# goldbricklemon/uplift-upsample-3dhpe

Measured on AMD Instinct MI355X. Metric: pose-sequences/sec, higher is better.
Workload: dtype f16x3 (f32 operands split into f16 hi/lo, 3 MFMA passes, f32 accumulate); 1 GPU; config/h36m_351.json forward, N=71 tokens (receptive field 351), J=17, batch 128/GPU, s_in=5, seeded Keras-default weights; global_batch=128, parallelism=batch-sharded x1, hipgraph=True, concurrent_half_batches=False, batches_in_flight=8

## Files before the change

uplift-upsample-3dhpe_amd/arch.py:

```python
import math
from dataclasses import dataclass, field
from typing import List, Tuple


@dataclass(frozen=True)
class UpliftArch:
    num_frames: int
    num_keypoints: int
    d_spatial: int
    d_temporal: int
    spatial_depth: int
    temporal_depth: int
    strides: Tuple[int, ...]
    paddings: Tuple[Tuple[int, int], ...]
    num_heads: int
    mlp_ratio: float
    qkv_bias: bool
    has_strided_input: bool
    first_strided_token_attention_layer: int
    full_output: bool
    drop_path_rate: Tuple[float, float, float]
    batch_size: int
    drop_rate: float = 0.0
    attention_drop_rate: float = 0.0
# ... 1 lines not shown
    learnable_masked_token: bool = False
    output_bn: bool = False
    strided_lengths: Tuple[int, ...] = field(default=())

    @property
    def h_spatial(self) -> int:
        return int(self.d_spatial * self.mlp_ratio)

    @property
    def h_temporal(self) -> int:
        return int(self.d_temporal * self.mlp_ratio)

    @property
    def out_dim(self) -> int:
        return 3 * self.num_keypoints

    @property
    def compiled_dims(self) -> bool:
        return (self.num_keypoints == 17 and self.d_spatial == 32 and self.h_spatial == 64 and self.num_heads == 8
                and self.d_temporal == 384)


def _pe_length_recurrence(n: int, strides, paddings) -> List[int]:
    out = [n]
    for s, p in zip(strides, paddings):
        out.append(math.ceil((out[-1] + p[0] + p[1] - 2) / s))
    return out


def _conv_length_recurrence(n: int, strides, paddings) -> List[int]:
    out = [n]
    for s, p in zip(strides, paddings):
        out.append((out[-1] + p[0] + p[1] - 3) // s + 1)
    return out


def training_unsupported(a: "UpliftArch"):
    out = []
    if not (0.0 <= a.drop_rate < 1.0):
        out.append(f"DROP_RATE = {a.drop_rate} (must be in [0, 1))")
    if not (0.0 <= a.attention_drop_rate < 1.0):
        out.append(f"ATTENTION_DROP_RATE = {a.attention_drop_rate} (must be in [0, 1))")
    return out


def arch_from_config(config) -> UpliftArch:
    has_strided_input = config.MASK_STRIDE is not None
    if has_strided_input:
        ms = config.MASK_STRIDE
        if type(ms) is int and ms == 1:
            has_strided_input = False
        if type(ms) is list and ms[0] == 1:
            has_strided_input = False

    strides = tuple(int(s) for s in config.STRIDES)
    if config.PADDINGS is None:
        paddings = tuple((1, 1) for _ in strides)
    else:
        paddings = tuple((int(p[0]), int(p[1])) for p in config.PADDINGS)
    if len(paddings) != len(strides):
        raise ValueError("PADDINGS must have one [left, right] pair per entry of STRIDES")

    n = int(config.SEQUENCE_LENGTH)
    pe_len = _pe_length_recurrence(n, strides, paddings)
    conv_len = _conv_length_recurrence(n, strides, paddings)
    if pe_len[:-1] != conv_len[:-1]:
# ... 68 lines not shown
```

uplift-upsample-3dhpe_amd/csrc/uu3d_api.hip:

```cpp
#include <hip/hip_runtime.h>

#include <algorithm>
#include <cmath>
#include <cstdio>
#include <cstdlib>
#include <cstring>
#include <functional>
#include <map>
#include <mutex>
#include <string>
#include <vector>

#include "../../include/uu3d.h"
#include "uu3d_switches.h"
#include "uu3d_gemm.h"
#include "uu3d_gemm_h3.h"
#include "uu3d_gemm_panel.h"
#include "uu3d_gemm_panel8.h"
#include "uu3d_gemm_wt.h"
#include "uu3d_mlp_fused.h"
#include "uu3d_tchain16.h"
#include "uu3d_attn.h"
#include "uu3d_attn_h3.h"
#include "uu3d_spatial.h"
// ... 37 lines not shown

struct WeightRec {
    std::string name;
    std::vector<int64_t> dims;
    int64_t numel = 0;
    std::vector<float> host;
    bool set = false;
};

struct BlockDev {
    const float *ln1_g, *ln1_b, *wqkv_t, *bqkv, *wp_t, *bp, *ln2_g, *ln2_b, *w1_t, *b1, *w2_t, *b2;
    const float* pe;
    size_t wqkv_pf = 0, w1_pf = 0;
    size_t w2_mf = 0;
    size_t wp_pf = 0;
};

struct ProfRec {
    std::string name, kernel;
    double flops, bytes;
    hipEvent_t e0, e1;
};

}

struct uu3d_train_state;
struct uu3d_model {
    uu3d_config cfg;
    uu3d_train_state* ts = nullptr;
    int device = 0;
    std::vector<WeightRec> weights;
    std::map<std::string, int> index;
    std::vector<int> L;
    Switches sw;
    bool committed = false;
    bool generic = false;
    float* gparams = nullptr;
    float* arena = nullptr;
    size_t arena_floats = 0;
    bool throughput = false;
    struct TcLaunch { int flags; size_t w_off ; size_t p_off ; };
    std::vector<TcLaunch> tchain;
    int num_cus = 256;
    std::recursive_mutex train_mu;
    bool in_commit = false;
    int* d_range = nullptr;
    _Float16* harena = nullptr;
    size_t harena_halfs = 0;
    std::map<size_t, std::pair<size_t, size_t>> hplanes;
    std::map<size_t, size_t> panel_off, mlpf_off;
    SpatialParams sp{};
    size_t sp_frag_off = 0;
    size_t sp_frag16_off = 0;
    const float *s2t_wt = nullptr, *s2t_b = nullptr, *token = nullptr, *pe_t = nullptr;
    std::vector<BlockDev> tblocks, sblocks;
    const float *h1_wt = nullptr, *h1_b = nullptr, *h2_wt = nullptr, *h2_b = nullptr;
    bool profiling = false;
    std::vector<ProfRec> prof;
    size_t prof_used = 0;
    std::string err;
};

namespace {

inline bool tchain_possible(const uu3d_config& c) {
    return c.precision == UU3D_PREC_F16X3 && c.d_temporal == 384 && c.h_temporal == 768 && c.num_heads == 8 && c.temporal_depth >= 1;
// ... 664 lines not shown
```

uplift-upsample-3dhpe_amd/csrc/uu3d_attn.h:

```cpp
#pragma once
#include <hip/hip_runtime.h>
#include <stdint.h>
#include <math.h>
#include "uu3d_gemm.h"

namespace uu3d {

typedef _Float16 h16x8v __attribute__((ext_vector_type(8)));
#ifdef UU3D_ATTN_STAMP
__device__ unsigned long long attn_clk[8];
#define ATTN_STAMP(...) __VA_ARGS__
#else
#define ATTN_STAMP(...)
#endif
template <int NT, int DH, bool SPLIT = false>
__global__ void __launch_bounds__(64 * NT)
attn_f32_kernel(const float* __restrict__ qkv, const int ld, const int D, const int L, const int H,
                const uint8_t* __restrict__ key_mask,
                float* __restrict__ out, const int ldo, const size_t lo_off = 0)
{
    static_assert(DH % 16 == 0, "head dim must be a multiple of 16");
    constexpr int LD = DH + 4;
    constexpr int F4 = DH / 4;
    constexpr int KT = DH / 16;
    constexpr int NS = (16 * F4 + 63) / 64;
    __shared__ __attribute__((aligned(16))) float Ks[NT * 16 * LD];
    __shared__ __attribute__((aligned(16))) float Vs[NT * 16 * LD];
    __shared__ __attribute__((aligned(16))) _Float16 Os[SPLIT ? NT : 1][SPLIT ? 2 * 16 * DH : 8];

    const int tid = threadIdx.x;
    const int lane = tid & 63, w = tid >> 6;
    const int qi = lane & 15, g = lane >> 4;
    const int qrow = 16 * w + qi;
    const int bh = ((int)gridDim.x & 7) == 0 ? ((int)blockIdx.x & 7) * ((int)gridDim.x >> 3) + ((int)blockIdx.x >> 3) : (int)blockIdx.x;

    const int b = bh / H, h = bh - b * H;
    float4 kreg[NS], vreg[NS];
    f32x4 qf[KT];
    {
        const float* base = qkv + (size_t)b * L * ld + h * DH;
#pragma unroll
        for (int s = 0; s < NS; ++s) {
            const int idx = tid + s * 64 * NT;
            const int row = idx / F4, c4 = (idx - row * F4) * 4;
            const float* p = base + (size_t)min(row, L - 1) * ld + c4;
            const float keep = (row < L) ? 1.0f : 0.0f;
            const float4 kv = *reinterpret_cast<const float4*>(p + D), vv = *reinterpret_cast<const float4*>(p + 2 * D);
            kreg[s] = make_float4(kv.x * keep, kv.y * keep, kv.z * keep, kv.w * keep);
            vreg[s] = make_float4(vv.x * keep, vv.y * keep, vv.z * keep, vv.w * keep);
        }
#pragma unroll
        for (int t = 0; t < KT; ++t)
            qf[t] = *reinterpret_cast<const f32x4*>(base + (size_t)min(qrow, L - 1) * ld + 16 * t + 4 * g);
    }
    ATTN_STAMP(const long long c0 = clock64();)
#pragma unroll
    for (int s = 0; s < NS; ++s) {
        const int idx = tid + s * 64 * NT;
        const int row = idx / F4, c4 = (idx - row * F4) * 4;
        if ((16 * F4) % 64 == 0 || idx < NT * 16 * F4) {
            *reinterpret_cast<float4*>(&Ks[row * LD + c4]) = kreg[s];
            *reinterpret_cast<float4*>(&Vs[row * LD + c4]) = vreg[s];
        }
    }
    __syncthreads();
    ATTN_STAMP(const long long c1 = clock64();)

    f32x4 st[NT];
#pragma unroll
    for (int j = 0; j < NT; ++j) {
        f32x4 a = (f32x4){0.f, 0.f, 0.f, 0.f};
// ... 46 lines not shown
    ATTN_STAMP(asm volatile("s_nop 0" :: "v"(st[NT - 1][3])); const long long c3 = clock64();)
    f32x4 ot[KT];
#pragma unroll
    for (int t = 0; t < KT; ++t) ot[t] = (f32x4){0.f, 0.f, 0.f, 0.f};
#pragma unroll
        for (int t = 0; t < KT; ++t)
#pragma unroll
            for (int j = 0; j < NT; ++j)
#pragma unroll
                for (int s = 0; s < 4; ++s) {
                    const float vv = Vs[(16 * j + 4 * g + s) * LD + 16 * t + qi];
                    ot[t] = __builtin_amdgcn_mfma_f32_16x16x4f32(st[j][s], vv, ot[t], 0, 0, 0);
                }
    if constexpr (SPLIT) {
        _Float16* Ow = Os[w];
#pragma unroll
        for (int t = 0; t < KT; ++t)
#pragma unroll
            for (int r = 0; r < 4; ++r) {
                const _Float16 hv = (fabsf(ot[t][r]) < 6.103515625e-05f) ? (_Float16)0.f : (_Float16)ot[t][r];
                const _Float16 lv = (_Float16)((ot[t][r] - (float)hv) * 2048.0f);
                Ow[(4 * g + r) * DH + 16 * t + qi] = hv;
                Ow[(16 + 4 * g + r) * DH + 16 * t + qi] = lv;
            }
        __builtin_amdgcn_fence(__ATOMIC_RELEASE, "wavefront");
        __builtin_amdgcn_wave_barrier();
        constexpr int PPR = DH / 8, PIECES = 2 * 16 * PPR;
        _Float16* oh = reinterpret_cast<_Float16*>(out);
#pragma unroll
        for (int i = 0; i < (PIECES + 63) / 64; ++i) {
            const int pc = lane + 64 * i;
            const int plane = pc / (16 * PPR), rem = pc - plane * 16 * PPR, row = rem / PPR, c8 = rem - row * PPR;
            const int q = 16 * w + row;
            if (pc < PIECES && q < L) {
                const h16x8v piece = *reinterpret_cast<const h16x8v*>(&Ow[(plane * 16 + row) * DH + 8 * c8]);
                const int grow = b * L + q, k = h * DH + 8 * c8;
                _Float16* dst = lo_off == 512 ? oh + ((size_t)(grow >> 5) * (size_t)(ldo >> 4) + (size_t)(k >> 4)) * 1024 + (size_t)plane * 512 + ((k >> 3) & 1) * 256 + (grow & 31) * 8
                                              : oh + (size_t)plane * lo_off + (size_t)grow * ldo + k;
                *reinterpret_cast<h16x8v*>(dst) = piece;
            }
        }
    } else {
#pragma unroll
        for (int t = 0; t < KT; ++t)
#pragma unroll
            for (int r = 0; r < 4; ++r) {
                const int q = 16 * w + 4 * g + r;
                if (q < L) out[((size_t)b * L + q) * ldo + h * DH + 16 * t + qi] = ot[t][r];
            }
    }
    ATTN_STAMP(asm volatile("s_waitcnt vmcnt(0)" ::: "memory"); if (tid == 0) { const long long c4 = clock64();
        atomicAdd(&attn_clk[0], (unsigned long long)(c1 - c0)); atomicAdd(&attn_clk[1], (unsigned long long)(c2 - c1));
        atomicAdd(&attn_clk[2], (unsigned long long)(c3 - c2)); atomicAdd(&attn_clk[3], (unsigned long long)(c4 - c3)); atomicAdd(&attn_clk[4], 1ull); })
}

template <int NT, int DH, bool SPLIT = false>
__global__ void __launch_bounds__(256, 1) __attribute__((amdgpu_waves_per_eu(1, 1)))
attn_head_wave_kernel(const float* __restrict__ qkv, const int ld, const int D, const int L, const int H,
                      const uint8_t* __restrict__ key_mask, float* __restrict__ out, const int ldo, const size_t lo_off, const int items)
{
    static_assert(DH % 16 == 0, "head dim must be a multiple of 16");
    constexpr int LD = DH + 4;
    constexpr int F4 = DH / 4;
    constexpr int KT = DH / 16;
    constexpr int NS = (NT * 16 * F4 + 63) / 64;
    constexpr int OS_HALFS = 2 * 16 * DH;
    extern __shared__ __attribute__((aligned(16))) float attn_lds[];
    const int tid = threadIdx.x, lane = tid & 63, w = tid >> 6;
    const int qi = lane & 15, g = lane >> 4;
    float* Ks = attn_lds + (size_t)w * 2 * NT * 16 * LD;
    float* Vs = Ks + NT * 16 * LD;
    _Float16* Os = reinterpret_cast<_Float16*>(attn_lds + (size_t)4 * 2 * NT * 16 * LD) + w * OS_HALFS;
    const int wg = ((int)gridDim.x & 7) == 0 ? ((int)blockIdx.x & 7) * ((int)gridDim.x >> 3) + ((int)blockIdx.x >> 3) : (int)blockIdx.x;
    const int bh = wg * 4 + w;
    if (bh >= items) return;
    size_t lo_off_s = lo_off; int ldo_s = ldo;
    asm volatile("" : "+s"(lo_off_s), "+s"(ldo_s));
    const int b = bh / H, h = bh - b * H;
    const float* base = qkv + (size_t)b * L * ld + h * DH;
    ATTN_STAMP(const long long c0 = clock64(); long long tqk = 0, tsm = 0, tpv = 0;)

    static_assert((NT * 16 * F4) % 64 == 0, "whole staging passes");
    {
        static_assert(NS <= 15, "the counted waits list at most 15 registers");
        f32x4 kx[15], vx[15];
        auto scalar_ptr = [](const float* q) {
// ... 179 lines not shown
```

uplift-upsample-3dhpe_amd/csrc/uu3d_commit.inc:

```
namespace {

struct Packer {
    std::vector<float> buf;
    std::vector<std::pair<size_t, size_t>> dense;
    size_t alloc(size_t n) {
        size_t off = align_up(buf.size(), 64);
        buf.resize(off + n, 0.f);
        return off;
    }
    size_t alloc_dense(size_t n) { const size_t off = alloc(n); dense.emplace_back(off, n); return off; }
};

const float* W(const uu3d_model* m, const std::string& name) {
    auto it = m->index.find(name);
    return it == m->index.end() ? nullptr : m->weights[it->second].host.data();
}

void pack_dense_t(std::vector<float>& buf, size_t off, const float* w, int K, int N, int Kp, int n0) {
    for (int k = 0; k < K; ++k)
        for (int n = 0; n < N; ++n) buf[off + (size_t)(n0 + n) * Kp + k] = w[(size_t)k * N + n];
}

}

int uu3d_commit_weights(uu3d_model* m, void* stream_) {
    if (!m) return UU3D_ERR_INVALID_ARGUMENT;
    for (auto& r : m->weights)
        if (!r.set) return fail(m, UU3D_ERR_NOT_READY, "weight never set: " + r.name);
    hipStream_t stream = (hipStream_t)stream_;
    HIPCHK(m, hipSetDevice(m->device));
    if (m->generic) {
        if (m->gparams == nullptr) {
            long long n = 0;
            for (auto& r : m->weights) n += r.numel;
            HIPCHK(m, hipMalloc((void**)&m->gparams, (size_t)n * sizeof(float)));
        }
        m->in_commit = true;
        const int r = uu3d_train_init(m, m->gparams, stream_);
        m->in_commit = false;
        if (r != UU3D_OK) return r;
        HIPCHK(m, hipStreamSynchronize(stream));
        m->committed = true;
        return UU3D_OK;
    }
    const uu3d_config& c = m->cfg;
    const int J = c.num_keypoints, N = c.num_frames, ds = c.d_spatial, dt = c.d_temporal, ht = c.h_temporal;
    const int Kdt = round_up(dt, 32), Kht = round_up(ht, 32), Ks2t = round_up(J * ds, 32);
    Packer P;

    const size_t o_ew = P.alloc(2 * ds), o_eb = P.alloc(ds), o_spe = P.alloc((size_t)J * ds);
    std::copy_n(W(m, "keypoint_embedding/kernel"), 2 * ds, P.buf.begin() + o_ew);
    std::copy_n(W(m, "keypoint_embedding/bias"), ds, P.buf.begin() + o_eb);
    std::copy_n(W(m, "spatial_pe/positional_encoding_weights"), J * ds, P.buf.begin() + o_spe);
// ... 292 lines not shown
                tchain16_reorder_mlp(tmp.data(), mlp);
            }
            m->tchain.push_back({tb.flags, at, tb.p_off});
        }
        if (m->harena_halfs < hb.size()) {
            if (m->harena) HIPCHK(m, hipFree(m->harena));
            m->harena = nullptr;
            HIPCHK(m, hipMalloc((void**)&m->harena, hb.size() * sizeof(_Float16)));
            m->harena_halfs = hb.size();
        }
        HIPCHK(m, hipMemcpyAsync(m->harena, hb.data(), hb.size() * sizeof(_Float16), hipMemcpyHostToDevice, stream));
        HIPCHK(m, hipStreamSynchronize(stream));
    }

    const float* A = m->arena;
    m->sp.embed_w = A + o_ew; m->sp.embed_b = A + o_eb; m->sp.pe = A + o_spe; m->sp.blocks = A + o_sblk;
    m->sp.norm_g = A + o_sng; m->sp.norm_b = A + o_snb; m->sp.depth = c.spatial_depth; m->sp.total_frames = 0;
    m->s2t_wt = A + o_s2t; m->s2t_b = A + o_s2tb; m->token = A + o_tok; m->pe_t = A + o_pet;
    auto view = [&](const BlockOff& o, bool strided) {
        BlockDev b{};
        b.ln1_g = A + o.ln1_g; b.ln1_b = A + o.ln1_b; b.wqkv_t = A + o.wqkv; b.bqkv = A + o.bqkv;
        b.wp_t = A + o.wp; b.bp = A + o.bp; b.ln2_g = A + o.ln2_g; b.ln2_b = A + o.ln2_b;
        b.w1_t = A + o.w1; b.b1 = A + o.b1; b.w2_t = A + o.w2; b.b2 = A + o.b2;
        b.pe = strided ? A + o.pe : nullptr;
        { const auto it = m->panel_off.find(o.wqkv); b.wqkv_pf = (it != m->panel_off.end()) ? it->second : 0; }
        { const auto it = m->panel_off.find(o.w1); b.w1_pf = (it != m->panel_off.end()) ? it->second : 0; }
        { const auto it = m->mlpf_off.find(o.w2); b.w2_mf = (!strided && it != m->mlpf_off.end()) ? it->second : 0; }
        { const auto it = m->panel_off.find(o.wp); b.wp_pf = (it != m->panel_off.end()) ? it->second : 0; }
        return b;
    };
    m->tblocks.clear(); m->sblocks.clear();
    for (auto& o : toff) m->tblocks.push_back(view(o, false));
    for (auto& o : soff) m->sblocks.push_back(view(o, true));
    m->h1_wt = has_h1 ? A + o_h1 : nullptr; m->h1_b = has_h1 ? A + o_h1b : nullptr;
    m->h2_wt = A + o_h2; m->h2_b = A + o_h2b;
    m->committed = true;
    return UU3D_OK;
}
```

uplift-upsample-3dhpe_amd/csrc/uu3d_forward.inc:

```

namespace {
struct Workspace {
    float *S, *X, *QKV, *O, *Hb, *XA, *XB, *slab, *mslab;
    unsigned char* tc_scratch;
    int* frame_list;
    float2* stats;
    size_t slab_floats;
    size_t bytes;
};
Workspace carve(const uu3d_model* m, int B, char* base) {
    const uu3d_config& c = m->cfg;
    const size_t rows = (size_t)B * c.num_frames;
    const size_t rows_s = (size_t)B * (c.num_strided > 1 ? std::max(m->L[1], 1) : 1);
    size_t off = 0;
    auto take = [&](size_t n) { size_t o = off; off = align_up(off + n, 256); return o; };
    Workspace w{};
    const size_t oS = take(rows * c.num_keypoints * c.d_spatial * 4);
    const size_t oX = take(rows * c.d_temporal * 4);
    const size_t oQ = take((rows + 128) * 3 * c.d_temporal * 4);
    const size_t oO = take((rows + 32) * c.d_temporal * 4);
    const size_t oH = take((rows + 32) * c.h_temporal * 4);
    const size_t oA = take(rows * c.d_temporal * 4);
    const size_t oB = take(rows_s * c.d_temporal * 4);
    const size_t oT = take(rows * sizeof(float2));
// ... 337 lines not shown
            if (nt <= 3) { if (mask) UU3D_ATTN_H3(3, 3, true, nt) else UU3D_ATTN_H3(3, 3, false, nt) }
            else if (nt <= 12) { if (mask) UU3D_ATTN_H3(12, 3, true, nt) else UU3D_ATTN_H3(12, 3, false, nt) }
            else { if (mask) UU3D_ATTN_H3(8, 2, true, std::min(nt, 8)) else UU3D_ATTN_H3(8, 2, false, std::min(nt, 8)) }
#undef UU3D_ATTN_H3
            end();
            return;
        }
        if (!m->sw.attn_wg && H % 4 == 0 && NT >= 4 && NT <= 5) {
            const dim3 hgrid((items + 3) / 4);
#define UU3D_ATTN_HW(nt) case nt: { \
            constexpr size_t lds = attn_head_wave_lds_bytes<nt, kDH>(); \
            if (split_lo_off) { allow_lds<attn_head_wave_kernel<nt, kDH, true>>(lds); \
                hipLaunchKernelGGL((attn_head_wave_kernel<nt, kDH, true>), hgrid, dim3(256), lds, stream, qkv, 3 * D, D, L, H, mask, out, D, frag ? (size_t)512 : split_lo_off, items); } \
            else { allow_lds<attn_head_wave_kernel<nt, kDH, false>>(lds); \
                hipLaunchKernelGGL((attn_head_wave_kernel<nt, kDH, false>), hgrid, dim3(256), lds, stream, qkv, 3 * D, D, L, H, mask, out, D, (size_t)0, items); } \
            } break;
            switch (NT) { UU3D_ATTN_HW(4) UU3D_ATTN_HW(5) default: break; }
#undef UU3D_ATTN_HW
            end();
            return;
        }
#define UU3D_ATTN_CASE(nt) case nt: \
        if (split_lo_off) hipLaunchKernelGGL((attn_f32_kernel<nt, kDH, true>), grid, dim3(64 * nt), 0, stream, qkv, 3 * D, D, L, H, mask, out, D, frag ? (size_t)512 : split_lo_off); \
        else hipLaunchKernelGGL((attn_f32_kernel<nt, kDH, false>), grid, dim3(64 * nt), 0, stream, qkv, 3 * D, D, L, H, mask, out, D, (size_t)0); \
        break;
        switch (NT) {
            UU3D_ATTN_CASE(1) UU3D_ATTN_CASE(2) UU3D_ATTN_CASE(3) UU3D_ATTN_CASE(4)
            UU3D_ATTN_CASE(5) UU3D_ATTN_CASE(6) UU3D_ATTN_CASE(7) UU3D_ATTN_CASE(8)
            default: status = UU3D_ERR_UNSUPPORTED; m->err = "attention over more than 128 tokens needs the f16x3 path (precision f16x3, d_t and h_t multiples of 32)"; break;
        }
#undef UU3D_ATTN_CASE
        end();
    }
};

template <class EP>
void spatial_stage(Launcher& Lh, const uu3d_config& c, const float* kp2d, int M, const uint8_t* mask, int* frame_list, float* S, bool timing_skip, const EP& ep) {
    uu3d_model* const m = Lh.m;
    const int J = c.num_keypoints, ds = c.d_spatial, dt = c.d_temporal;
    const bool h3 = c.precision == UU3D_PREC_F16X3 && !m->sw.spatial_f32 && (m->sw.spatial_h3_always || spatial_h3_pays(M));
    const bool planes = h3 && !m->sw.no_planes && (J * ds) % 32 == 0;
    const bool skip = timing_skip && (skip_mask() & 1);
    SpatialParams sp = m->sp;
    sp.total_frames = M;
    sp.frame_list = nullptr;
    if (mask != nullptr) {
        Lh.begin("compact_frames", "compact_frames", 0.0, (double)M * 5.0);
        hipLaunchKernelGGL(compact_frames_kernel, dim3(1), dim3(1024), 0, Lh.stream, mask, M, frame_list);
        Lh.end();
        sp.frame_list = frame_list;
    }
    const double fl = (double)M * (2.0 * J * 2 * ds + c.spatial_depth * (4.0 * 2 * J * ds * ds + 8.0 * 4 * J * J * (ds / 8) + 2.0 * 2 * J * ds * kHS));
    _Float16* const s_hi = planes ? reinterpret_cast<_Float16*>(S) : (_Float16*)nullptr;
    _Float16* const s_lo = planes ? reinterpret_cast<_Float16*>(S) + (size_t)M * J * ds : (_Float16*)nullptr;
    if (h3 && m->sw.spatial_h3_tiles) {
        Lh.begin("spatial_stack", "spatial_h3", fl, 4.0 * M * J * (2.0 + ds));
        if (!skip)
        hipLaunchKernelGGL((spatial_stack_h3_kernel<kJ, kFR, kSpatialMT>), dim3((M + kFR - 1) / kFR), dim3(64 * (2 / kSpatialMT)), sh3::lds_bytes(), Lh.stream, kp2d, sp,
                           m->harena + m->sp_frag_off, S, s_hi, s_lo, SpatialTrainIO{});
        Lh.end();
    } else if (h3) {
        Lh.begin("spatial_stack", "spatial_p16", fl, 4.0 * M * J * (2.0 + ds));
        if (!skip)
        hipLaunchKernelGGL((spatial_stack_p16_kernel<kJ, kP16FR, kP16PW>), dim3((M + kP16FR - 1) / kP16FR), dim3(64 * p16_waves(kJ, kP16FR, kP16PW)), sp16::lds_bytes<kP16FR>(c.spatial_depth),
                           Lh.stream, kp2d, sp, m->harena + m->sp_frag16_off, S, s_hi, s_lo);
        Lh.end();
// ... 27 lines not shown

struct Forward {
    uu3d_model* const m;
    Launcher Lh;
    const Workspace w;
    const uu3d_config c;
    const uint8_t* const mask;
    const int B;
    float* const full_out; float* const central_out; float* const* const attn_out;
    const bool part_body, part_tail;

    const int N = c.num_frames, J = c.num_keypoints, dt = c.d_temporal, ht = c.h_temporal, M = B * N;
    const bool has_h1 = c.full_output && c.temporal_depth > 0;
    const bool planes = (c.precision == UU3D_PREC_F16X3) && (dt % 32 == 0) && (ht % 32 == 0) && !m->sw.no_planes;
    const bool chain = Lh.throughput && planes && m->sw.tchain_mode != 0 && (m->sw.tchain_mode == 1 || (M + 127) / 128 >= m->sw.tchain_min_tiles) && !m->tchain.empty() && M >= 1024 &&
                       (Lh.attn_is_h3(N, true) || (m->sw.tchain_short && Lh.attn_h3_any(N))) && (c.num_strided == 0 || m->L[0] == N) && (double)M * 1152 * 4.0 < 4.0e9 &&
                       attn_out == nullptr;
    _Float16* const Ph = reinterpret_cast<_Float16*>(w.O);
    _Float16* const Hh = reinterpret_cast<_Float16*>(w.Hb);
    const BlockDev* pend = nullptr;
    float* xa = w.XA;
    char nm[48];

    void tokens_from_frames(const FramesIn& frames) {
        Lh.begin("frames_to_tokens", "frames_to_tokens", 0.0, 4.0 * 3.0 * M * dt);
        hipLaunchKernelGGL(frames_to_tokens_kernel, dim3((unsigned)(((size_t)M * (dt / 4) + 255) / 256)), dim3(256), 0, Lh.stream,
                           frames.features, frames.num_rows, frames.rows, mask, m->token, m->pe_t, (long)M, N, dt, w.X);
        Lh.end();
    }
    void spatial(const float* kp2d) {
        spatial_stage(Lh, c, kp2d, M, mask, w.frame_list, w.S, true, EpSpatialToTemporal{w.X, m->s2t_b, dt, mask, m->token, m->pe_t, N});
    }

    const _Float16* block_head(const char* tag, int i, const BlockDev& b, float* x, int L, const uint8_t* kmask, const BlockDev* prev, bool fuse_mlp) {
        const int Mr = B * L;
        auto name = [&](const char* what) { snprintf(nm, sizeof nm, "%s%d.%s", tag, i + 1, what); return nm; };
        _Float16* const Pl = Ph + (size_t)Mr * dt; _Float16* const Hl = Hh + (size_t)Mr * ht;
        const bool qsplit = Lh.attn_is_h3(L, planes);
        _Float16* const Qh = reinterpret_cast<_Float16*>(w.QKV); _Float16* const Ql = Qh + (size_t)Mr * 3 * dt;
        const EpBiasSplitQ ep_qs{Qh, Ql, b.bqkv, 3 * dt, dt, Lh.attn_qscale()};
        const bool few = planes && Mr <= kFewRows && Lh.wt_ok(b.wqkv_t, dt) && Lh.wt_ok(b.w1_t, dt);
        auto maps = [&]() {
            if (attn_out != nullptr && tag[0] == 't' && attn_out[i] != nullptr) {
                Lh.begin(name("attn_maps"), "attn_probs", 2.0 * B * (double)c.num_heads * L * L * kDH, 4.0 * B * (double)c.num_heads * L * L);
                const size_t lds = (size_t)L * (kDH + 1) * sizeof(float);
                allow_lds<attn_probs_kernel>(160 * 1024 - 256);
                if (qsplit) hipLaunchKernelGGL(attn_probs_kernel, dim3(B * c.num_heads), dim3(256), lds, Lh.stream, (const void*)Qh, (const _Float16*)Ql, 3 * dt, dt, L, c.num_heads, kDH, kmask, 1.0f, 1, attn_out[i]);
                else hipLaunchKernelGGL(attn_probs_kernel, dim3(B * c.num_heads), dim3(256), lds, Lh.stream, (const void*)w.QKV, (const _Float16*)nullptr, 3 * dt, dt, L, c.num_heads, kDH, kmask, 1.0f / sqrtf((float)kDH), 0, attn_out[i]);
                Lh.end();
            }
        };
        if (few) {
            WtLoadF32 l1{x, dt, Mr, dt, b.ln1_g, b.ln1_b, 1e-5f, 1};
            if (qsplit) Lh.gemm_wt(name("ln_qkv"), l1, b.wqkv_t, Mr, 3 * dt, dt, ep_qs);
            else Lh.gemm_wt(name("ln_qkv"), l1, b.wqkv_t, Mr, 3 * dt, dt, EpBias{w.QKV, b.bqkv, 3 * dt});
            maps();
            Lh.attn(name("attn"), w.QKV, B, L, kmask, w.O, (size_t)Mr * dt);
            { GLoadPlain gl{Ph, Pl, dt, Mr}; Lh.gemm_g(name("proj_res"), gl, b.wp_t, Mr, dt, dt, EpBiasResidual{x, b.bp, dt, nullptr, nullptr, 1}, 4.0 * Mr * dt); }
            WtLoadF32 l2{x, dt, Mr, dt, b.ln2_g, b.ln2_b, 1e-5f, 1};
            Lh.gemm_wt(name("ln_fc1"), l2, b.w1_t, Mr, ht, dt, EpBiasReluSplit{Hh, Hl, b.b1, ht});
            return nullptr;
        }
        if (prev != nullptr) {
            if (x == w.X) Lh.ln_res_split_frag(name("ln1_split"), w.X, Mr, prev->b2, w.mslab, nullptr, nullptr, 1, b.ln1_g, b.ln1_b, Ph);
            else Lh.ln_res_split_frag(name("ln1_split"), w.X, Mr, prev->b2, w.mslab, x, b.pe, L, b.ln1_g, b.ln1_b, Ph);
            if (qsplit) Lh.gemm_panel(name("ln_qkv"), Ph, b.wqkv_pf, b.bqkv, Mr, 3 * dt, PanelEpBiasSplitQ{Qh, Ql, 3 * dt, dt, Lh.attn_qscale()});
            else Lh.gemm_panel(name("ln_qkv"), Ph, b.wqkv_pf, b.bqkv, Mr, 3 * dt, PanelEpBias{w.QKV, 3 * dt});
        } else if (planes && Lh.panel_ok(Mr, 3 * dt, dt, b.wqkv_pf)) {
            Lh.ln_split_frag(name("ln1_split"), x, Mr, b.ln1_g, b.ln1_b, Ph);
            if (qsplit) Lh.gemm_panel(name("ln_qkv"), Ph, b.wqkv_pf, b.bqkv, Mr, 3 * dt, PanelEpBiasSplitQ{Qh, Ql, 3 * dt, dt, Lh.attn_qscale()});
            else Lh.gemm_panel(name("ln_qkv"), Ph, b.wqkv_pf, b.bqkv, Mr, 3 * dt, PanelEpBias{w.QKV, 3 * dt});
        } else {
            Lh.row_stats(name("stats1"), x, dt, Mr, w.stats);
            ALoadLayerNorm al{x, w.stats, b.ln1_g, b.ln1_b, dt, Mr, dt};
            if (qsplit) Lh.gemm(name("ln_qkv"), al, b.wqkv_t, Mr, 3 * dt, dt, ep_qs);
            else { EpBias ep{w.QKV, b.bqkv, 3 * dt}; Lh.gemm(name("ln_qkv"), al, b.wqkv_t, Mr, 3 * dt, dt, ep); }
        }
        maps();
        const bool pproj = planes && !m->sw.no_panel_proj && Lh.panel_ok(Mr, dt, dt, b.wp_pf);
        Lh.attn(name("attn"), w.QKV, B, L, kmask, w.O, planes ? (size_t)Mr * dt : 0, pproj);
        const bool mlp_panel = planes && Lh.panel_ok(Mr, ht, dt, b.w1_pf);
        bool ln2_done = false;
        if (pproj) ln2_done = mlp_panel ? Lh.gemm_panel_residual(name("proj_res"), Ph, b.wp_pf, b.bp, Mr, x, b.ln2_g, b.ln2_b, Ph)
                                        : Lh.gemm_panel_residual(name("proj_res"), Ph, b.wp_pf, b.bp, Mr, x);
        else {
            EpBiasResidual ep{x, b.bp, dt, nullptr, nullptr, 1};
            if (planes) { GLoadPlain gl{Ph, Pl, dt, Mr}; Lh.gemm_g(name("proj_res"), gl, b.wp_t, Mr, dt, dt, ep, 4.0 * Mr * dt); }
            else { ALoadPlain al{w.O, dt, Mr, dt}; Lh.gemm(name("proj_res"), al, b.wp_t, Mr, dt, dt, ep, 4.0 * Mr * dt); }
        }
        if (mlp_panel) {
            if (!ln2_done) Lh.ln_split_frag(name("ln2_split"), x, Mr, b.ln2_g, b.ln2_b, Ph);
            if (fuse_mlp) return Ph;
            Lh.gemm_panel(name("ln_fc1"), Ph, b.w1_pf, b.b1, Mr, ht, PanelEpBiasReluSplit{Hh, Hl, ht});
        } else {
            Lh.row_stats(name("stats2"), x, dt, Mr, w.stats);
            ALoadLayerNorm al{x, w.stats, b.ln2_g, b.ln2_b, dt, Mr, dt};
            if (planes) { EpBiasReluSplit ep{Hh, Hl, b.b1, ht}; Lh.gemm(name("ln_fc1"), al, b.w1_t, Mr, ht, dt, ep); }
            else { EpBiasRelu ep{w.Hb, b.b1, ht}; Lh.gemm(name("ln_fc1"), al, b.w1_t, Mr, ht, dt, ep); }
        }
        return nullptr;
    }

    void temporal_chain() {
        _Float16* const Q = reinterpret_cast<_Float16*>(w.QKV);
        Lh.tchain("t1.ln_qkv", m->tchain[0], M, nullptr, w.X, nullptr, nullptr, 1, Q, nullptr, w.tc_scratch);
        for (int i = 0; i < c.temporal_depth; ++i) {
            const bool masked = c.has_strided_input && i < c.first_strided_token_attention_layer;
            snprintf(nm, sizeof nm, "t%d.attn", i + 1);
            Lh.attn(nm, w.QKV, B, N, masked ? mask : nullptr, w.O, (size_t)M * dt, true, true);
            const bool to_strided = i + 1 == c.temporal_depth && c.num_strided > 0;
            snprintf(nm, sizeof nm, "t%d.chain", i + 1);
            Lh.tchain(nm, m->tchain[i + 1], M, Ph, w.X, to_strided ? w.XA : nullptr, to_strided ? m->sblocks[0].pe : nullptr, N, Q, nullptr, w.tc_scratch);
        }
    }
    void temporal_blocks() {
        for (int i = 0; i < c.temporal_depth; ++i) {
            const BlockDev& b = m->tblocks[i];
            const bool masked = c.has_strided_input && i < c.first_strided_token_attention_layer;
            const bool last = (i + 1 == c.temporal_depth);
            const bool fuse = planes && Lh.mlpf_ok(M, b) && (last ? (c.num_strided > 0 && Lh.panel_ok(M, 3 * dt, dt, m->sblocks[0].wqkv_pf))
                                                                  : Lh.panel_ok(M, 3 * dt, dt, m->tblocks[i + 1].wqkv_pf));
            const _Float16* const a2 = block_head("t", i, b, w.X, N, masked ? mask : nullptr, pend, fuse);
            pend = nullptr;
            if (fuse) {
                snprintf(nm, sizeof nm, "t%d.mlp", i + 1);
                Lh.mlp_fused(nm, a2, b, M, w.mslab);
                pend = &b;
                continue;
            }
            const bool to_strided = last && c.num_strided > 0;
            EpBiasResidual ep_fc2{w.X, b.b2, dt, to_strided ? w.XA : nullptr, to_strided ? m->sblocks[0].pe : nullptr, N};
            snprintf(nm, sizeof nm, "t%d.fc2_res", i + 1);
            if (planes) { GLoadPlain gl{Hh, Hh + (size_t)M * ht, ht, M}; Lh.gemm_g(nm, gl, b.w2_t, M, dt, ht, ep_fc2, 4.0 * M * dt); }
            else { ALoadPlain al{w.Hb, ht, M, ht}; Lh.gemm(nm, al, b.w2_t, M, dt, ht, ep_fc2, 4.0 * M * dt); }
        }
    }
    void head1() {
        if (!has_h1) return;
        ALoadPlain al{w.X, dt, M, dt}; EpBias ep{full_out, m->h1_b, 3 * J};
        Lh.gemm("head1", al, m->h1_wt, M, 3 * J, dt, ep);
    }
    void strided_blocks() {
        float* xb = w.XB;
        const _Float16* const hzero = m->harena;
        if (c.temporal_depth == 0 && c.num_strided > 0) {
            Lh.begin("s1.add_pe", "add_pe", 0.0, 12.0 * M * dt);
            hipLaunchKernelGGL(add_period_kernel, dim3((unsigned)(((size_t)M * dt / 4 + 255) / 256)), dim3(256), 0, Lh.stream, w.X, m->sblocks[0].pe, M, dt, N, w.XA);
            Lh.end();
        }
        for (int i = 0; i < c.num_strided; ++i) {
            const BlockDev& b = m->sblocks[i];
            const int Li = m->L[i], Lo = m->L[i + 1], Mi = B * Li, Mo = B * Lo;
            if (((skip_mask() & 256) || part_body) && i >= 1) continue;
            if (((skip_mask() & 512) || part_tail) && i == 0) { std::swap(xa, xb); xb = w.XA; continue; }
            const int lo = (c.strides[i] > 1 && c.pad_left[i] == 0) ? 1 : 0;
            const EpConvResidual ep_conv{xb, b.b2, dt, xa, Li, Lo, c.strides[i], lo,
                                         (i + 1 < c.num_strided) ? m->sblocks[i + 1].pe : nullptr};
            const bool smask = c.temporal_depth == 0 && c.has_strided_input && i < c.first_strided_token_attention_layer;
            if (chain && i == 0) {
                Lh.attn("s1.attn", w.QKV, B, Li, nullptr, w.O, (size_t)Mi * dt, true, true);
                Lh.tchain("s1.chain", m->tchain[c.temporal_depth + 1], Mi, Ph, nullptr, xa, nullptr, 1, nullptr, Hh, w.tc_scratch);
            } else
            block_head("s", i, b, xa, Li, smask ? mask : nullptr, i == 0 ? pend : nullptr, false);
            if (i == 0) head1();
            snprintf(nm, sizeof nm, "s%d.conv_res", i + 1);
            if (planes) { GLoadConv3 gl{Hh, Hh + (size_t)Mi * ht, hzero, ht, Li, Lo, c.strides[i], c.pad_left[i], Mo};
                          Lh.gemm_g(nm, gl, b.w2_t, Mo, dt, 3 * ht, ep_conv, 4.0 * Mo * dt); }
            else { ALoadConv3 al{w.Hb, ht, Li, Lo, c.strides[i], c.pad_left[i], Mo, 3 * ht};
                   Lh.gemm(nm, al, b.w2_t, Mo, dt, 3 * ht, ep_conv, 4.0 * Mo * dt); }
            std::swap(xa, xb);
            if (i == 0) xb = w.XA;
        }
    }
    void head2() {
        ALoadPlain al{c.num_strided > 0 ? xa : w.X + (size_t)(N / 2) * dt, c.num_strided > 0 ? dt : N * dt, B, dt};
        EpBias ep{central_out, m->h2_b, 3 * J};
        Lh.gemm("head2", al, m->h2_wt, B, 3 * J, dt, ep);
    }
    void range_check() {
        if (c.precision != UU3D_PREC_F16X3) return;
        Lh.begin("range_check", "range_check", 0.0, 4.0 * ((has_h1 ? (double)M * 3 * J : 0.0) + (double)B * 3 * J));
        hipLaunchKernelGGL(range_check_kernel, dim3(256), dim3(256), 0, Lh.stream, has_h1 ? full_out : central_out, has_h1 ? (long)M * 3 * J : 0L,
                           central_out, (long)B * 3 * J, m->d_range);
        Lh.end();
    }
};

int forward_impl(uu3d_model* m, const float* kp2d, const FramesIn* frames, const uint8_t* mask, int32_t B, float* full_out,
                 float* central_out, float* const* attn_out, void* workspace, size_t workspace_bytes, int32_t schedule, void* stream_) {
    if (!m) return UU3D_ERR_INVALID_ARGUMENT;
    const bool exact_f32 = (schedule & UU3D_SCHEDULE_EXACT_F32) != 0;
    schedule &= ~UU3D_SCHEDULE_EXACT_F32;
#ifdef UU3D_TIMING_BUILD
    const bool parts_ok = process_switches().timing_parts;
#else
    constexpr bool parts_ok = false;
#endif
    const bool part_body = parts_ok && (schedule & 0x200) != 0, part_tail = parts_ok && (schedule & 0x400) != 0;
    if (parts_ok) schedule &= ~0x600;
// ... 110 lines not shown
```

uplift-upsample-3dhpe_amd/csrc/uu3d_switches.h:

```cpp
#pragma once
#include <cstdio>
#include <cstdlib>
#include <string>

namespace uu3d {

struct Switches {
    bool spatial_f32 = false;
    bool spatial_h3_always = false;
    bool spatial_h3_tiles = false;
    bool no_planes = false;
    bool attn_wg = false;
    bool no_mlpf = false;
    bool no_wt = false;
    bool attn_f32 = false;
    bool no_panel = false;
    bool no_panel_proj = false;
    int tchain_mode = -1;
    int tchain_min_tiles = 8;
    bool tchain_short = true;
    struct Train {
        bool f32 = false;
        bool one_stream = false;
        bool event_flags_set = false;
        unsigned event_flags = 0;
        bool any_queue = false;
        bool spatial_unfused = false;
        bool no_panel = false;
        bool attn_bwd_generic = false;
    } train;
};

inline Switches read_switches() {
    Switches s;
    auto is1 = [](const char* name) { const char* e = getenv(name); return e != nullptr && e[0] == '1'; };
    auto present = [](const char* name) { return getenv(name) != nullptr; };
    { const char* e = getenv("UU3D_SPATIAL"); const std::string v = e ? e : "";
      s.spatial_f32 = v == "f32"; s.spatial_h3_always = v == "h3"; s.spatial_h3_tiles = v == "h3tiles"; }
    s.no_planes = is1("UU3D_NO_PLANES");
    s.attn_wg = is1("UU3D_ATTN_WG");
    s.no_mlpf = is1("UU3D_NO_MLPF");
    s.no_wt = is1("UU3D_NO_WT");
    s.attn_f32 = is1("UU3D_ATTN_F32");
    s.no_panel = is1("UU3D_NO_PANEL");
    s.no_panel_proj = is1("UU3D_NO_PANEL_PROJ");
    { const char* e = getenv("UU3D_TCHAIN"); if (e != nullptr && (e[0] == '0' || e[0] == '1')) s.tchain_mode = e[0] - '0'; }
    { const char* e = getenv("UU3D_TCHAIN_MIN_TILES"); if (e != nullptr && atoi(e) > 0) s.tchain_min_tiles = atoi(e); }
    { const char* e = getenv("UU3D_TCHAIN_SHORT"); if (e != nullptr) s.tchain_short = atoi(e) != 0; }
    s.train.f32 = present("UU3D_TRAIN_F32");
    s.train.one_stream = present("UU3D_TRAIN_1STREAM");
    { const char* e = getenv("UU3D_TRAIN_EVENT_FLAGS"); s.train.event_flags_set = e != nullptr; if (e) s.train.event_flags = (unsigned)strtoul(e, nullptr, 0); }
    s.train.any_queue = present("UU3D_TRAIN_ANY_QUEUE");
    s.train.spatial_unfused = present("UU3D_TRAIN_SPATIAL_UNFUSED");
    s.train.no_panel = present("UU3D_TRAIN_NO_PANEL");
    s.train.attn_bwd_generic = present("UU3D_ATTN_BWD_GENERIC");
    return s;
}

struct ProcessSwitches {
#ifdef UU3D_TIMING_BUILD
    int skip = 0;
    bool timing_parts = false;
#endif
    bool panel4 = false;
    int panel_s = 0;
    int panel_proj_s = 0;
    bool no_ln_tail = false;
    int thr_splitk_target = 192;
    int tnh_wgs = 192;
    int gemm_deep_wgs = 640;
    bool tn_f32 = false;
    bool capture_inorder = false;
};

inline const ProcessSwitches& process_switches() {
    static const ProcessSwitches sw = [] {
        ProcessSwitches s;
#ifdef UU3D_TIMING_BUILD
        { const char* e = getenv("UU3D_SKIP"); s.skip = e ? atoi(e) : 0;
          if (s.skip) fprintf(stderr, "[uu3d] UU3D_SKIP=%d: launches are being skipped, RESULTS ARE WRONG (timing experiment)\n", s.skip); }
        { const char* e = getenv("UU3D_TIMING_PARTS"); s.timing_parts = e != nullptr && atoi(e) != 0; }
// ... 17 lines not shown
```

Baseline: 216,600 pose-sequences/s.

## Compute only conv-tapped rows after attention in strided transformer blocks

For strided blocks after the first, where the stride-3 conv reads only a subset of token rows, attention writes output just for the live rows. Those rows are compacted into a smaller buffer, and the residual input is compacted alongside. The proj, LN2, fc1 and conv-residual GEMMs then run on fewer rows, and the conv loader is remapped to a dense stride-3 layout. This cuts GEMM work in the later strided blocks, at the cost of extra gather/scatter logic in the attention kernel and a more complex indexing path.

```diff
diff --git a/uplift-upsample-3dhpe_amd/arch.py b/uplift-upsample-3dhpe_amd/arch.py
--- a/uplift-upsample-3dhpe_amd/arch.py
+++ b/uplift-upsample-3dhpe_amd/arch.py
@@ -57,6 +57,20 @@
     out = [n]
     for s, p in zip(strides, paddings):
         out.append((out[-1] + p[0] + p[1] - 3) // s + 1)
+    return out
+
+
+def strided_live_rows(a: "UpliftArch") -> List[List[int]]:
+    out = []
+    L = a.strided_lengths
+    for i, (s, p) in enumerate(zip(a.strides, a.paddings)):
+        li, lo, pl = L[i], L[i + 1], p[0]
+        last = s * (lo - 1) - pl + 2
+        taps = [s * o + j - pl for o in range(lo) for j in range(3) if 0 <= s * o + j - pl < li]
+        if i == 0 or s < 3 or pl > 1 or last > li or li > 48 or 4 * len(taps) > 3 * li:
+            out.append(list(range(li)))
+        else:
+            out.append(taps)
     return out
 
 
diff --git a/uplift-upsample-3dhpe_amd/csrc/uu3d_api.hip b/uplift-upsample-3dhpe_amd/csrc/uu3d_api.hip
--- a/uplift-upsample-3dhpe_amd/csrc/uu3d_api.hip
+++ b/uplift-upsample-3dhpe_amd/csrc/uu3d_api.hip
@@ -93,6 +93,7 @@
     std::vector<WeightRec> weights;
     std::map<std::string, int> index;
     std::vector<int> L;
+    std::vector<int> Llive;
     Switches sw;
     bool committed = false;
     bool generic = false;
diff --git a/uplift-upsample-3dhpe_amd/csrc/uu3d_attn.h b/uplift-upsample-3dhpe_amd/csrc/uu3d_attn.h
--- a/uplift-upsample-3dhpe_amd/csrc/uu3d_attn.h
+++ b/uplift-upsample-3dhpe_amd/csrc/uu3d_attn.h
@@ -13,12 +13,30 @@
 #else
 #define ATTN_STAMP(...)
 #endif
-template <int NT, int DH, bool SPLIT = false>
-__global__ void __launch_bounds__(64 * NT)
-attn_f32_kernel(const float* __restrict__ qkv, const int ld, const int D, const int L, const int H,
-                const uint8_t* __restrict__ key_mask,
-                float* __restrict__ out, const int ldo, const size_t lo_off = 0)
+struct AttnRowsAll {
+    static constexpr bool kLive = false;
+    __device__ __forceinline__ int rows(int L) const { return L; }
+    __device__ __forceinline__ int pos(int q) const { return q; }
+};
+struct AttnRowsLive {
+    static constexpr bool kLive = true;
+    int stride, pad, Lc;
+    const float* __restrict__ x; float* __restrict__ xc;
+    __device__ __forceinline__ int rows(int) const { return Lc; }
+    __device__ __forceinline__ int pos(int q) const {
+        const int t = q + pad, o = t / stride, j = t - o * stride, r = 3 * o + j - pad;
+        return (j < 3 && r >= 0 && r < Lc) ? r : -1;
+    }
+    __device__ __forceinline__ int token(int r) const { const int t = r + pad, o = t / 3; return o * stride + (t - 3 * o) - pad; }
+};
+
+template <int NT, int DH, bool SPLIT, class ROWS>
+__device__ __forceinline__ void
+attn_f32_body(const float* __restrict__ qkv, const int ld, const int D, const int L, const int H,
+              const uint8_t* __restrict__ key_mask,
+              float* __restrict__ out, const int ldo, const size_t lo_off, const ROWS rows)
 {
+    static_assert(!ROWS::kLive || SPLIT, "live rows leave as f16 planes");
     static_assert(DH % 16 == 0, "head dim must be a multiple of 16");
     constexpr int LD = DH + 4;
     constexpr int F4 = DH / 4;
@@ -37,6 +55,16 @@
     const int b = bh / H, h = bh - b * H;
     float4 kreg[NS], vreg[NS];
     f32x4 qf[KT];
+    const int Lr = rows.rows(L);
+    float4 xreg[ROWS::kLive ? NS : 1];
+    if constexpr (ROWS::kLive) {
+#pragma unroll
+        for (int s = 0; s < NS; ++s) {
+            const int idx = tid + s * 64 * NT;
+            const int r = min(idx / F4, Lr - 1), c4 = (idx - (idx / F4) * F4) * 4;
+            xreg[s] = *reinterpret_cast<const float4*>(rows.x + ((size_t)b * L + rows.token(r)) * ldo + h * DH + c4);
+        }
+    }
     {
         const float* base = qkv + (size_t)b * L * ld + h * DH;
 #pragma unroll
@@ -149,9 +177,10 @@
             const int pc = lane + 64 * i;
             const int plane = pc / (16 * PPR), rem = pc - plane * 16 * PPR, row = rem / PPR, c8 = rem - row * PPR;
             const int q = 16 * w + row;
-            if (pc < PIECES && q < L) {
+            const int qp = rows.pos(q);
+            if (pc < PIECES && q < L && qp >= 0) {
                 const h16x8v piece = *reinterpret_cast<const h16x8v*>(&Ow[(plane * 16 + row) * DH + 8 * c8]);
-                const int grow = b * L + q, k = h * DH + 8 * c8;
+                const int grow = b * Lr + qp, k = h * DH + 8 * c8;
                 _Float16* dst = lo_off == 512 ? oh + ((size_t)(grow >> 5) * (size_t)(ldo >> 4) + (size_t)(k >> 4)) * 1024 + (size_t)plane * 512 + ((k >> 3) & 1) * 256 + (grow & 31) * 8
                                               : oh + (size_t)plane * lo_off + (size_t)grow * ldo + k;
                 *reinterpret_cast<h16x8v*>(dst) = piece;
@@ -166,9 +195,32 @@
                 if (q < L) out[((size_t)b * L + q) * ldo + h * DH + 16 * t + qi] = ot[t][r];
             }
     }
+    if constexpr (ROWS::kLive) {
+#pragma unroll
+        for (int s = 0; s < NS; ++s) {
+            const int idx = tid + s * 64 * NT;
+            const int r = idx / F4, c4 = (idx - r * F4) * 4;
+            if (r < Lr) *reinterpret_cast<float4*>(rows.xc + ((size_t)b * Lr + r) * ldo + h * DH + c4) = xreg[s];
+        }
+    }
     ATTN_STAMP(asm volatile("s_waitcnt vmcnt(0)" ::: "memory"); if (tid == 0) { const long long c4 = clock64();
         atomicAdd(&attn_clk[0], (unsigned long long)(c1 - c0)); atomicAdd(&attn_clk[1], (unsigned long long)(c2 - c1));
         atomicAdd(&attn_clk[2], (unsigned long long)(c3 - c2)); atomicAdd(&attn_clk[3], (unsigned long long)(c4 - c3)); atomicAdd(&attn_clk[4], 1ull); })
+}
+
+template <int NT, int DH, bool SPLIT = false>
+__global__ void __launch_bounds__(64 * NT)
+attn_f32_kernel(const float* __restrict__ qkv, const int ld, const int D, const int L, const int H,
+                const uint8_t* __restrict__ key_mask, float* __restrict__ out, const int ldo, const size_t lo_off = 0)
+{
+    attn_f32_body<NT, DH, SPLIT>(qkv, ld, D, L, H, key_mask, out, ldo, lo_off, AttnRowsAll{});
+}
+template <int NT, int DH>
+__global__ void __launch_bounds__(64 * NT)
+attn_live_kernel(const float* __restrict__ qkv, const int ld, const int D, const int L, const int H,
+                 const uint8_t* __restrict__ key_mask, float* __restrict__ out, const int ldo, const size_t lo_off, const AttnRowsLive rows)
+{
+    attn_f32_body<NT, DH, true>(qkv, ld, D, L, H, key_mask, out, ldo, lo_off, rows);
 }
 
 template <int NT, int DH, bool SPLIT = false>
diff --git a/uplift-upsample-3dhpe_amd/csrc/uu3d_commit.inc b/uplift-upsample-3dhpe_amd/csrc/uu3d_commit.inc
--- a/uplift-upsample-3dhpe_amd/csrc/uu3d_commit.inc
+++ b/uplift-upsample-3dhpe_amd/csrc/uu3d_commit.inc
@@ -19,6 +19,14 @@
 void pack_dense_t(std::vector<float>& buf, size_t off, const float* w, int K, int N, int Kp, int n0) {
     for (int k = 0; k < K; ++k)
         for (int n = 0; n < N; ++n) buf[off + (size_t)(n0 + n) * Kp + k] = w[(size_t)k * N + n];
+}
+
+int live_rows(const uu3d_config& c, const std::vector<int>& L, int i) {
+    const int Li = L[i], Lo = L[i + 1], s = c.strides[i], pl = c.pad_left[i];
+    const int last = s * (Lo - 1) - pl + 2;
+    if (i == 0 || s < 3 || pl > 1 || last > Li || Li > 48) return Li;
+    const int Lc = 3 * Lo - pl - (last == Li ? 1 : 0);
+    return 4 * Lc <= 3 * Li ? Lc : Li;
 }
 
 }
@@ -377,6 +385,8 @@
     m->tblocks.clear(); m->sblocks.clear();
     for (auto& o : toff) m->tblocks.push_back(view(o, false));
     for (auto& o : soff) m->sblocks.push_back(view(o, true));
+    m->Llive.clear();
+    for (int i = 0; i < c.num_strided; ++i) m->Llive.push_back(m->sw.strided_live ? live_rows(c, m->L, i) : m->L[i]);
     m->h1_wt = has_h1 ? A + o_h1 : nullptr; m->h1_b = has_h1 ? A + o_h1b : nullptr;
     m->h2_wt = A + o_h2; m->h2_b = A + o_h2b;
     m->committed = true;
diff --git a/uplift-upsample-3dhpe_amd/csrc/uu3d_forward.inc b/uplift-upsample-3dhpe_amd/csrc/uu3d_forward.inc
--- a/uplift-upsample-3dhpe_amd/csrc/uu3d_forward.inc
+++ b/uplift-upsample-3dhpe_amd/csrc/uu3d_forward.inc
@@ -393,6 +393,20 @@
 #undef UU3D_ATTN_CASE
         end();
     }
+    void attn_live(const char* name, const float* qkv, int B, int L, int Lc, int stride, int pad_left, const uint8_t* mask, float* out, bool frag, const float* x, float* xc) {
+        if (skip_mask() & 16) return;
+        const int D = m->cfg.d_temporal, H = m->cfg.num_heads, NT = (L + 15) / 16;
+        begin(name, "attn_live", 4.0 * B * (double)H * L * L * kDH, 4.0 * B * D * (3.0 * L + 3.0 * Lc));
+        const AttnRowsLive rows{stride, pad_left, Lc, x, xc};
+        const size_t lo_off = frag ? (size_t)512 : (size_t)B * Lc * D;
+#define UU3D_ATTN_LIVE(nt) case nt: hipLaunchKernelGGL((attn_live_kernel<nt, kDH>), dim3(B * H), dim3(64 * nt), 0, stream, qkv, 3 * D, D, L, H, mask, out, D, lo_off, rows); break;
+        switch (NT) {
+            UU3D_ATTN_LIVE(1) UU3D_ATTN_LIVE(2) UU3D_ATTN_LIVE(3)
+            default: status = UU3D_ERR_UNSUPPORTED; m->err = "attn_live: more than 48 tokens"; break;
+        }
+#undef UU3D_ATTN_LIVE
+        end();
+    }
 };
 
 template <class EP>
@@ -486,14 +500,23 @@
         spatial_stage(Lh, c, kp2d, M, mask, w.frame_list, w.S, true, EpSpatialToTemporal{w.X, m->s2t_b, dt, mask, m->token, m->pe_t, N});
     }
 
-    const _Float16* block_head(const char* tag, int i, const BlockDev& b, float* x, int L, const uint8_t* kmask, const BlockDev* prev, bool fuse_mlp) {
+    const _Float16* block_head(const char* tag, int i, const BlockDev& b, float* x, int L, const uint8_t* kmask, const BlockDev* prev, bool fuse_mlp,
+                               int Lc = 0, int conv_stride = 0, int conv_pad = 0, float* xc = nullptr) {
         const int Mr = B * L;
+        const bool live = Lc > 0 && Lc < L;
+        const int Mt = live ? B * Lc : Mr;
+        float* const xt = live ? xc : x;
         auto name = [&](const char* what) { snprintf(nm, sizeof nm, "%s%d.%s", tag, i + 1, what); return nm; };
-        _Float16* const Pl = Ph + (size_t)Mr * dt; _Float16* const Hl = Hh + (size_t)Mr * ht;
+        _Float16* const Pl = Ph + (size_t)Mt * dt; _Float16* const Hl = Hh + (size_t)Mt * ht;
         const bool qsplit = Lh.attn_is_h3(L, planes);
         _Float16* const Qh = reinterpret_cast<_Float16*>(w.QKV); _Float16* const Ql = Qh + (size_t)Mr * 3 * dt;
         const EpBiasSplitQ ep_qs{Qh, Ql, b.bqkv, 3 * dt, dt, Lh.attn_qscale()};
-        const bool few = planes && Mr <= kFewRows && Lh.wt_ok(b.wqkv_t, dt) && Lh.wt_ok(b.w1_t, dt);
+        auto few_rows = [&](int rows) { return planes && rows <= kFewRows && Lh.wt_ok(b.wqkv_t, dt) && Lh.wt_ok(b.w1_t, dt); };
+        const bool few = few_rows(Mr);
+        auto attention = [&](bool frag) {
+            if (live) Lh.attn_live(name("attn"), w.QKV, B, L, Lc, conv_stride, conv_pad, kmask, w.O, frag, x, xt);
+            else Lh.attn(name("attn"), w.QKV, B, L, kmask, w.O, planes ? (size_t)Mr * dt : 0, frag);
+        };
         auto maps = [&]() {
             if (attn_out != nullptr && tag[0] == 't' && attn_out[i] != nullptr) {
                 Lh.begin(name("attn_maps"), "attn_probs", 2.0 * B * (double)c.num_heads * L * L * kDH, 4.0 * B * (double)c.num_heads * L * L);
@@ -508,14 +531,7 @@
             WtLoadF32 l1{x, dt, Mr, dt, b.ln1_g, b.ln1_b, 1e-5f, 1};
             if (qsplit) Lh.gemm_wt(name("ln_qkv"), l1, b.wqkv_t, Mr, 3 * dt, dt, ep_qs);
             else Lh.gemm_wt(name("ln_qkv"), l1, b.wqkv_t, Mr, 3 * dt, dt, EpBias{w.QKV, b.bqkv, 3 * dt});
-            maps();
-            Lh.attn(name("attn"), w.QKV, B, L, kmask, w.O, (size_t)Mr * dt);
-            { GLoadPlain gl{Ph, Pl, dt, Mr}; Lh.gemm_g(name("proj_res"), gl, b.wp_t, Mr, dt, dt, EpBiasResidual{x, b.bp, dt, nullptr, nullptr, 1}, 4.0 * Mr * dt); }
-            WtLoadF32 l2{x, dt, Mr, dt, b.ln2_g, b.ln2_b, 1e-5f, 1};
-            Lh.gemm_wt(name("ln_fc1"), l2, b.w1_t, Mr, ht, dt, EpBiasReluSplit{Hh, Hl, b.b1, ht});
-            return nullptr;
-        }
-        if (prev != nullptr) {
+        } else if (prev != nullptr) {
             if (x == w.X) Lh.ln_res_split_frag(name("ln1_split"), w.X, Mr, prev->b2, w.mslab, nullptr, nullptr, 1, b.ln1_g, b.ln1_b, Ph);
             else Lh.ln_res_split_frag(name("ln1_split"), w.X, Mr, prev->b2, w.mslab, x, b.pe, L, b.ln1_g, b.ln1_b, Ph);
             if (qsplit) Lh.gemm_panel(name("ln_qkv"), Ph, b.wqkv_pf, b.bqkv, Mr, 3 * dt, PanelEpBiasSplitQ{Qh, Ql, 3 * dt, dt, Lh.attn_qscale()});
@@ -531,26 +547,33 @@
             else { EpBias ep{w.QKV, b.bqkv, 3 * dt}; Lh.gemm(name("ln_qkv"), al, b.wqkv_t, Mr, 3 * dt, dt, ep); }
         }
         maps();
-        const bool pproj = planes && !m->sw.no_panel_proj && Lh.panel_ok(Mr, dt, dt, b.wp_pf);
-        Lh.attn(name("attn"), w.QKV, B, L, kmask, w.O, planes ? (size_t)Mr * dt : 0, pproj);
-        const bool mlp_panel = planes && Lh.panel_ok(Mr, ht, dt, b.w1_pf);
+        if (few_rows(Mt)) {
+            attention(false);
+            { GLoadPlain gl{Ph, Pl, dt, Mt}; Lh.gemm_g(name("proj_res"), gl, b.wp_t, Mt, dt, dt, EpBiasResidual{xt, b.bp, dt, nullptr, nullptr, 1}, 4.0 * Mt * dt); }
+            WtLoadF32 l2{xt, dt, Mt, dt, b.ln2_g, b.ln2_b, 1e-5f, 1};
+            Lh.gemm_wt(name("ln_fc1"), l2, b.w1_t, Mt, ht, dt, EpBiasReluSplit{Hh, Hl, b.b1, ht});
+            return nullptr;
+        }
+        const bool pproj = planes && !m->sw.no_panel_proj && Lh.panel_ok(Mt, dt, dt, b.wp_pf);
+        attention(pproj);
+        const bool mlp_panel = planes && Lh.panel_ok(Mt, ht, dt, b.w1_pf);
         bool ln2_done = false;
-        if (pproj) ln2_done = mlp_panel ? Lh.gemm_panel_residual(name("proj_res"), Ph, b.wp_pf, b.bp, Mr, x, b.ln2_g, b.ln2_b, Ph)
-                                        : Lh.gemm_panel_residual(name("proj_res"), Ph, b.wp_pf, b.bp, Mr, x);
+        if (pproj) ln2_done = mlp_panel ? Lh.gemm_panel_residual(name("proj_res"), Ph, b.wp_pf, b.bp, Mt, xt, b.ln2_g, b.ln2_b, Ph)
+                                        : Lh.gemm_panel_residual(name("proj_res"), Ph, b.wp_pf, b.bp, Mt, xt);
         else {
-            EpBiasResidual ep{x, b.bp, dt, nullptr, nullptr, 1};
-            if (planes) { GLoadPlain gl{Ph, Pl, dt, Mr}; Lh.gemm_g(name("proj_res"), gl, b.wp_t, Mr, dt, dt, ep, 4.0 * Mr * dt); }
-            else { ALoadPlain al{w.O, dt, Mr, dt}; Lh.gemm(name("proj_res"), al, b.wp_t, Mr, dt, dt, ep, 4.0 * Mr * dt); }
+            EpBiasResidual ep{xt, b.bp, dt, nullptr, nullptr, 1};
+            if (planes) { GLoadPlain gl{Ph, Pl, dt, Mt}; Lh.gemm_g(name("proj_res"), gl, b.wp_t, Mt, dt, dt, ep, 4.0 * Mt * dt); }
+            else { ALoadPlain al{w.O, dt, Mt, dt}; Lh.gemm(name("proj_res"), al, b.wp_t, Mt, dt, dt, ep, 4.0 * Mt * dt); }
         }
         if (mlp_panel) {
-            if (!ln2_done) Lh.ln_split_frag(name("ln2_split"), x, Mr, b.ln2_g, b.ln2_b, Ph);
+            if (!ln2_done) Lh.ln_split_frag(name("ln2_split"), xt, Mt, b.ln2_g, b.ln2_b, Ph);
             if (fuse_mlp) return Ph;
-            Lh.gemm_panel(name("ln_fc1"), Ph, b.w1_pf, b.b1, Mr, ht, PanelEpBiasReluSplit{Hh, Hl, ht});
+            Lh.gemm_panel(name("ln_fc1"), Ph, b.w1_pf, b.b1, Mt, ht, PanelEpBiasReluSplit{Hh, Hl, ht});
         } else {
-            Lh.row_stats(name("stats2"), x, dt, Mr, w.stats);
-            ALoadLayerNorm al{x, w.stats, b.ln2_g, b.ln2_b, dt, Mr, dt};
-            if (planes) { EpBiasReluSplit ep{Hh, Hl, b.b1, ht}; Lh.gemm(name("ln_fc1"), al, b.w1_t, Mr, ht, dt, ep); }
-            else { EpBiasRelu ep{w.Hb, b.b1, ht}; Lh.gemm(name("ln_fc1"), al, b.w1_t, Mr, ht, dt, ep); }
+            Lh.row_stats(name("stats2"), xt, dt, Mt, w.stats);
+            ALoadLayerNorm al{xt, w.stats, b.ln2_g, b.ln2_b, dt, Mt, dt};
+            if (planes) { EpBiasReluSplit ep{Hh, Hl, b.b1, ht}; Lh.gemm(name("ln_fc1"), al, b.w1_t, Mt, ht, dt, ep); }
+            else { EpBiasRelu ep{w.Hb, b.b1, ht}; Lh.gemm(name("ln_fc1"), al, b.w1_t, Mt, ht, dt, ep); }
         }
         return nullptr;
     }
@@ -608,17 +631,19 @@
             if (((skip_mask() & 256) || part_body) && i >= 1) continue;
             if (((skip_mask() & 512) || part_tail) && i == 0) { std::swap(xa, xb); xb = w.XA; continue; }
             const int lo = (c.strides[i] > 1 && c.pad_left[i] == 0) ? 1 : 0;
-            const EpConvResidual ep_conv{xb, b.b2, dt, xa, Li, Lo, c.strides[i], lo,
+            const bool live = planes && i >= 1 && m->Llive[i] < Li;
+            const int Lt = live ? m->Llive[i] : Li, Mt = B * Lt, st = live ? 3 : c.strides[i], pl = c.pad_left[i];
+            const EpConvResidual ep_conv{xb, b.b2, dt, live ? w.X : xa, Lt, Lo, st, lo,
                                          (i + 1 < c.num_strided) ? m->sblocks[i + 1].pe : nullptr};
             const bool smask = c.temporal_depth == 0 && c.has_strided_input && i < c.first_strided_token_attention_layer;
             if (chain && i == 0) {
                 Lh.attn("s1.attn", w.QKV, B, Li, nullptr, w.O, (size_t)Mi * dt, true, true);
                 Lh.tchain("s1.chain", m->tchain[c.temporal_depth + 1], Mi, Ph, nullptr, xa, nullptr, 1, nullptr, Hh, w.tc_scratch);
             } else
-            block_head("s", i, b, xa, Li, smask ? mask : nullptr, i == 0 ? pend : nullptr, false);
+            block_head("s", i, b, xa, Li, smask ? mask : nullptr, i == 0 ? pend : nullptr, false, Lt, c.strides[i], pl, w.X);
             if (i == 0) head1();
             snprintf(nm, sizeof nm, "s%d.conv_res", i + 1);
-            if (planes) { GLoadConv3 gl{Hh, Hh + (size_t)Mi * ht, hzero, ht, Li, Lo, c.strides[i], c.pad_left[i], Mo};
+            if (planes) { GLoadConv3 gl{Hh, Hh + (size_t)Mt * ht, hzero, ht, Lt, Lo, st, pl, Mo};
                           Lh.gemm_g(nm, gl, b.w2_t, Mo, dt, 3 * ht, ep_conv, 4.0 * Mo * dt); }
             else { ALoadConv3 al{w.Hb, ht, Li, Lo, c.strides[i], c.pad_left[i], Mo, 3 * ht};
                    Lh.gemm(nm, al, b.w2_t, Mo, dt, 3 * ht, ep_conv, 4.0 * Mo * dt); }
diff --git a/uplift-upsample-3dhpe_amd/csrc/uu3d_switches.h b/uplift-upsample-3dhpe_amd/csrc/uu3d_switches.h
--- a/uplift-upsample-3dhpe_amd/csrc/uu3d_switches.h
+++ b/uplift-upsample-3dhpe_amd/csrc/uu3d_switches.h
@@ -19,6 +19,7 @@
     int tchain_mode = -1;
     int tchain_min_tiles = 8;
     bool tchain_short = true;
+    bool strided_live = true;
     struct Train {
         bool f32 = false;
         bool one_stream = false;
@@ -47,6 +48,7 @@
     { const char* e = getenv("UU3D_TCHAIN"); if (e != nullptr && (e[0] == '0' || e[0] == '1')) s.tchain_mode = e[0] - '0'; }
     { const char* e = getenv("UU3D_TCHAIN_MIN_TILES"); if (e != nullptr && atoi(e) > 0) s.tchain_min_tiles = atoi(e); }
     { const char* e = getenv("UU3D_TCHAIN_SHORT"); if (e != nullptr) s.tchain_short = atoi(e) != 0; }
+    { const char* e = getenv("UU3D_STRIDED_LIVE"); if (e != nullptr) s.strided_live = atoi(e) != 0; }
     s.train.f32 = present("UU3D_TRAIN_F32");
     s.train.one_stream = present("UU3D_TRAIN_1STREAM");
     { const char* e = getenv("UU3D_TRAIN_EVENT_FLAGS"); s.train.event_flags_set = e != nullptr; if (e) s.train.event_flags = (unsigned)strtoul(e, nullptr, 0); }
```

Result: no change. 218,200 pose-sequences/s (median of 6 runs) (+0.7%).
